# tu-darmstadt-ros-pkg/hector_slam

Measured on AMD Instinct MI355X. Metric: scan-match GN iterations/sec (1081-beam, 2048^2 map), higher is better.
Workload: dtype f32; 1 GPU; configs[2]: batch=4096/GPU concurrent 1081-beam scans (distinct pose+scan pairs), 2048^2 map, 1-level matchData = 6 GN it/scan, starts +-0.15 m / +-0.05 rad (SURVEY 8(d)); batch_per_gpu=4096, global_batch=4096, beams=1081, map=2048, levels=1, parallelism=dp1, parity_mode=library default (HSM_PARITY_AUTO) -> exact summation for this launch, parity_effective=exact

## Files before the change

hector_slam_amd/csrc/gn_match_exact.h:

```cpp
#pragma once
#include "gn_match.h"

namespace hsm {

constexpr int kXRow = 64 + kExactPad;

#ifndef HSM_XBPC
#define HSM_XBPC 15
#endif
#ifndef HSM_XBPC_MAIN
#define HSM_XBPC_MAIN 13
#endif
#ifndef HSM_XBPC_CW
#define HSM_XBPC_CW 6
#endif
constexpr int kXRows = 9;
#ifndef HSM_XOWNER_PRIO_P
#define HSM_XOWNER_PRIO_P 1
#endif
#ifndef HSM_XOWNER_SHIFT
#define HSM_XOWNER_SHIFT 8
#endif
#ifndef HSM_XEP_AHEAD
#define HSM_XEP_AHEAD 2
#endif
#ifndef HSM_XJOB_PRIO
#define HSM_XJOB_PRIO 3
#endif

#ifdef HSM_XTIMELINE
#define HSM_XT(row, slot)                                                                                            \
  do {                                                                                                               \
    if (P.clock_probe != nullptr && blockIdx.x == 0 && lane == 0)                                                    \
      P.clock_probe[((size_t)wave * BPL + (size_t)(row)) * 4 + (slot)] = (unsigned long long)__builtin_readcyclecounter(); \
  } while (0)
#else
#define HSM_XT(row, slot) \
  do {                    \
  } while (0)
#endif

__device__ __forceinline__ void set_prio_uniform(int p) {
  if (p <= 0) __builtin_amdgcn_s_setprio(0);
  else if (p == 1) __builtin_amdgcn_s_setprio(1);
  else if (p == 2) __builtin_amdgcn_s_setprio(2);
  else __builtin_amdgcn_s_setprio(3);
}

template <int NS, int BPL, int BPC = BPL, bool CW = false, bool PROBE = false>
__global__ void __launch_bounds__(64 * (NS + (CW ? 1 : 0)), CW && 5 * BPC + 50 <= 96 ? 5 : 4) gn_match_exact_cached_kernel(const MatchParams P) {
  static_assert(BPC >= 1 && BPC <= BPL, "cached rows are a prefix of the rows");
  constexpr int NC = 9 * NS;
  static_assert(!CW || NC <= 64, "the chain wavefront runs one job per round: lane = chain");
  constexpr int NCP = NC >= 64 ? NC : 64;
  constexpr int NB = NCP % 64 == 0 ? 2 : 3;
  constexpr int kLdsShare = 160 * 1024 / (16 / NS);
  constexpr int kRowsFit = (kLdsShare - NB * NS * kXRows * kXRow * 4 - NC * 4 - 64) / (NS * 512);
  constexpr int RV = BPL <= kRowsFit ? 0 : BPL - kRowsFit;
  static_assert(RV < BPL && RV <= 8, "endpoint rows kept in VGPRs");
  static_assert(64 * (NS + (CW ? 1 : 0)) <= 1024, "one workgroup");
  struct alignas(16) Smem {
    float stage[NB][NS][kXRows][kXRow];
    float runs[NC];
    int nmax;
    f2 pts[NS][BPL - RV][64];
  };
  static_assert(sizeof(Smem) <= kLdsShare, "16 wavefronts per CU");
  __shared__ Smem sm;
  auto& stage = sm.stage;
  auto& runs = sm.runs;
  int& nmax_s = sm.nmax;
  auto& lds_pts = sm.pts;
  static_assert(sizeof(sm.stage) < 65536, "stage rows are addressed through M0[15:0]");
  const int match_blocks = (!CW && P.xp.world > 0) ? P.xp.match_blocks : (int)gridDim.x;
  if (!CW && (int)blockIdx.x >= match_blocks) {
    exchange_wait_unpack(P.xp, (int)blockIdx.x - match_blocks);
    return;
  }
  const int lane = threadIdx.x & 63;
  const int wave = __builtin_amdgcn_readfirstlane((int)(threadIdx.x >> 6));
  const int slot = __builtin_amdgcn_readfirstlane(xcd_block((int)blockIdx.x, match_blocks, P.xcd_chunk) * NS + wave);
  const int scan = (P.perm != nullptr && slot < P.batch) ? __builtin_amdgcn_readfirstlane(P.perm[slot]) : slot;
  const bool chain_wave = CW && wave == NS;
  const bool active = slot < P.batch && !chain_wave;
  int beg = 0, n = 0;
  float pw0 = 0.0f, pw1 = 0.0f, pw2 = 0.0f;
  if (active) {
    n = P.shared_n;
    if (P.offsets) {
      beg = P.offsets[scan];
      n = P.offsets[scan + 1] - beg;
    }
    pw0 = P.begin_world[3 * scan + 0];
    pw1 = P.begin_world[3 * scan + 1];
    pw2 = P.begin_world[3 * scan + 2];
  }
  pw0 = uniform_f32(pw0), pw1 = uniform_f32(pw1), pw2 = uniform_f32(pw2);
  const float b0 = pw0, b1 = pw1, b2 = pw2;
  if (threadIdx.x == 0) nmax_s = 0;
  __syncthreads();
  if (lane == 0 && n > 0) atomicMax(&nmax_s, n);
  __syncthreads();
  const int nmax = nmax_s;
  if (nmax == 0) {
    if (!CW && active && P.xp.world > 0) exchange_post_pose(P.xp, scan, b0, b1, b2);
    if (active && lane == 0) {
      P.out_pose[3 * scan + 0] = b0;
      P.out_pose[3 * scan + 1] = b1;
      P.out_pose[3 * scan + 2] = b2;
    }
    return;
  }
  const int rounds = BPL + (nmax > 64 * BPL ? (nmax - 64 * BPL + 63) >> 6 : 0);
  const int units = rounds * NCP;
  if (CW && chain_wave) {
    __builtin_amdgcn_s_setprio(HSM_XJOB_PRIO);
    const int c = lane < NC ? lane : 0;
    for (int l = P.first_level; l >= P.last_level; --l) {
      const int gn_steps = __builtin_amdgcn_readfirstlane(P.lv[l].gn_steps);
      for (int it = 0; it < gn_steps; ++it) {
        float run = 0.0f;
        for (int k = 0; k < rounds; ++k) {
          asm volatile("s_waitcnt lgkmcnt(0)\n\ts_barrier" ::: "memory");
          const f4v* pa = reinterpret_cast<const f4v*>(&stage[0][0][0][0] + ((k % NB) * NC + c) * kXRow);
          f4v a[4];
#pragma unroll
          for (int q = 0; q < 4; ++q) a[q] = pa[q];
#pragma unroll
          for (int h = 0; h < 8; ++h) {
            const f4v p0 = a[2 * (h & 1)], p1 = a[2 * (h & 1) + 1];
            run += p0.x;
            run += p0.y;
            run += p0.z;
            run += p0.w;
            run += p1.x;
            run += p1.y;
            run += p1.z;
            run += p1.w;
            asm volatile("" : "+v"(run) : : "memory");
            if (h + 2 < 8) a[2 * (h & 1)] = pa[2 * h + 4], a[2 * (h & 1) + 1] = pa[2 * h + 5];
            asm volatile("" ::: "memory");
          }
        }
        if (lane < NC) runs[lane] = run;
        asm volatile("s_waitcnt lgkmcnt(0)\n\ts_barrier" ::: "memory");
      }
    }
    return;
  }
  const unsigned long long probe_t0 = PROBE ? (unsigned long long)__builtin_readcyclecounter() : 0ull;
  const unsigned long long probe_w0 = PROBE ? wall_clock64() : 0ull;
#ifdef HSM_XTIMELINE_WG
  if (P.clock_probe != nullptr && wave == 0 && lane == 0) {
    P.clock_probe[1024 + 4 * (size_t)blockIdx.x + 0] = wall_clock64();
    unsigned xcc;
    asm volatile("s_getreg_b32 %0, hwreg(HW_REG_XCC_ID)" : "=s"(xcc));
    unsigned hwid;
    asm volatile("s_getreg_b32 %0, hwreg(HW_REG_HW_ID)" : "=s"(hwid));
    P.clock_probe[1024 + 4 * (size_t)blockIdx.x + 2] = ((unsigned long long)xcc << 32) | hwid;
  }
#endif
  const float2* __restrict__ pts = P.pts + (n > 0 ? beg : 0);
  f2(*mine)[64] = lds_pts[wave];
  f2 pv[RV > 0 ? RV : 1];
  constexpr int kEpAhead = HSM_XEP_AHEAD < BPL ? HSM_XEP_AHEAD : BPL - 1;
  static_assert(BPL <= 31, "PeelSchedule holds 32 positions per load kind");
  constexpr PeelSchedule kSched = peel_schedule(BPL, kEpAhead);
  const bool peel = P.lv[P.first_level].gn_steps > 0;
  if (!peel) {
#pragma unroll
    for (int k = 0; k < BPL; ++k) {
      const int i = lane + 64 * k;
      const float2 q = i < n ? pts[i] : make_float2(1.0e30f, 1.0e30f);
      if (k < RV)
        pv[k] = f2{q.x, q.y};
      else
        mine[k - RV][lane] = f2{q.x, q.y};
    }
  }
  f4v tq[BPC];
  unsigned toff[BPC];
  Acc9 acc;
  acc.zero();
  float reg_scale = 1.0f;
  int step_no = 0;
  const int owner_phase = (int)((blockIdx.x >> HSM_XOWNER_SHIFT) & 3u);
  const unsigned st_wave = __builtin_amdgcn_readfirstlane((unsigned)(size_t)&stage[0][wave][0][0]);
  for (int l = P.first_level; l >= P.last_level; --l) {
    const LevelView& L = P.lv[l];
    float ex, ey, eth;
    affine_apply(L.mapTworld, pw0, pw1, ex, ey);
    ex = uniform_f32(ex), ey = uniform_f32(ey);
    eth = pw2;
    const float ps = L.pt_scale;
    const int gn_steps = L.gn_steps;
    const LevelRegs R = level_regs<kLayoutQuad>(L);
    const float ratio = ps / reg_scale;
    reg_scale = ps;
    const bool peel_here = peel && l == P.first_level;
#pragma unroll
    for (int k = 0; k < BPL; ++k) {
      if (!peel_here && ratio != 1.0f) {
        if (k < RV)
          pv[k] *= f2{ratio, ratio};
        else
          mine[k - RV][lane] *= f2{ratio, ratio};
      }
      if (k < BPC) toff[k] = 0xffffffffu;
    }
    unsigned zero_off = (unsigned)R.zero_index << 4;
    asm volatile("" : "+v"(zero_off));
    auto gn_step = [&](auto FIRST) {
      constexpr bool kFirst = decltype(FIRST)::value;
#ifdef HSM_XTIMELINE_STEPS
      if (P.clock_probe != nullptr && blockIdx.x == 0 && wave == 0 && lane == 0 && step_no < 32)
        P.clock_probe[(size_t)4 * 31 * 4 + step_no] = (unsigned long long)__builtin_readcyclecounter();
#endif
      f2 pq[kFirst ? BPL : 1];
      auto endpoint_issue = [&](int k) {
        int i = max(min((int)lane_id_now() + 64 * k, n - 1), 0);
        asm volatile("" : "+v"(i));
        const unsigned byte_off = (unsigned)i << 3;
        asm volatile("global_load_dwordx2 %0, %1, %2" : "=v"(pq[kFirst ? k : 0]) : "v"(byte_off), "s"(pts) : "memory");
      };
      if (kFirst) {
#pragma unroll
        for (int k = 0; k <= kEpAhead; ++k) endpoint_issue(k);
      }
      float sinRot, cosRot;
      sincos_f32<true>(eth, sinRot, cosRot);
      const f2 o2 = step_origin(ex, ey);
      const f2 e2 = f2{uniform_f32(o2.x), uniform_f32(o2.y)};
      const f2 cs = f2{uniform_f32(cosRot), uniform_f32(sinRot)}, sc = f2{cs.y, cs.x};
      auto endpoint = [&](int k) -> f2 {
        if (kFirst) {
          wait_vmcnt(kSched.posG[k] - kSched.posE[k] - 1, pq[kFirst ? k : 0]);
          const bool pad = (int)lane_id_now() + 64 * k >= n;
          const f2 q = pq[kFirst ? k : 0];
          const f2 p = f2{(pad ? 1.0e30f : q.x) * ps, (pad ? 1.0e30f : q.y) * ps};
          if (k < RV)
            pv[k < RV ? k : 0] = p;
          else
            mine[k < RV ? 0 : k - RV][lane] = p;
          return p;
        }
        return k < RV ? pv[k < RV ? k : 0] : mine[k < RV ? 0 : k - RV][lane];
      };
      f4v tu[2];
      auto locate = [&](int k, f2 p, BeamRot& r, float& fx, float& fy) {
        r.r.x = cs.x * p.x - sc.x * p.y;
        r.r.y = cs.y * p.x + sc.y * p.y;
        const CellCoord q = cell_coord(R, f2{e2.x + r.r.x, e2.y + r.r.y});
        fx = q.fx;
        fy = q.fy;
        unsigned idx = quad_index(q.ix, q.iy, R.tiles_x, R.sx);
        asm volatile("" : "+v"(idx));
        const unsigned off = q.oob ? zero_off : idx << 4;
        if (k >= BPC) {
          asm volatile("global_load_dwordx4 %[t], %[o], %[b]" : [t] "=v"(tu[k & 1]) : [o] "v"(off), [b] "s"(R.quad) : "memory");
          return;
        }
        const int kc = k < BPC ? k : 0;
        if (kFirst) {
          asm volatile("global_load_dwordx4 %[t], %[o], %[b]" : [t] "=v"(tq[kc]) : [o] "v"(off), [b] "s"(R.quad) : "memory");
          toff[kc] = off;
          return;
        }
        unsigned long long saved;
        asm volatile(
            "v_cmp_ne_u32 vcc, %[o], %[to]\n\t"
            "s_or_b32 vcc_lo, vcc_lo, 1\n\t"
            "s_and_saveexec_b64 %[sv], vcc\n\t"
            "global_load_dwordx4 %[t], %[o], %[b]\n\t"
            "v_mov_b32 %[to], %[o]\n\t"
            "s_mov_b64 exec, %[sv]"
            : [t] "+v"(tq[kc]), [to] "+v"(toff[kc]), [sv] "=&s"(saved)
            : [o] "v"(off), [b] "s"(R.quad)
            : "vcc", "scc", "memory");
      };
      auto texel_ready = [&](int k, bool has_next) {
        f4v& tx = k < BPC ? tq[k < BPC ? k : 0] : tu[k & 1];
        if (kFirst) {
          wait_vmcnt((has_next ? kSched.posG[k + 1] + 1 : kSched.total) - kSched.posG[k] - 1, tx);
        } else if (has_next) {
          asm volatile("s_waitcnt vmcnt(1)" : "+v"(tx) : : "memory");
        } else {
          asm volatile("s_waitcnt vmcnt(0)" : "+v"(tx) : : "memory");
        }
      };
      auto beam_terms4 = [&](float i0, float i1, float i2, float i3, const BeamRot& r, float fx, float fy, float (&tm)[4]) {
        const float xFacInv = 1.0f - fx, yFacInv = 1.0f - fy;
        const float M = ((i0 * xFacInv + i1 * fx) * (yFacInv)) + ((i2 * xFacInv + i3 * fx) * (fy));
        tm[0] = ((i1 - i0) * xFacInv) + ((i3 - i2) * fx);
        tm[1] = ((i2 - i0) * yFacInv) + ((i3 - i1) * fy);
        tm[2] = 1.0f - M;
        tm[3] = r.r.x * tm[1] - r.r.y * tm[0];
      };
      auto products_of = [&](const float (&tm)[4], float (&pp)[9]) {
        const float gx = tm[0], gy = tm[1], funVal = tm[2], rotDeriv = tm[3];
        pp[0] = gx * funVal, pp[1] = gy * funVal, pp[2] = rotDeriv * funVal;
        pp[3] = gx * gx, pp[4] = gy * gy, pp[5] = rotDeriv * rotDeriv;
        pp[6] = gx * gy, pp[7] = gx * rotDeriv, pp[8] = gy * rotDeriv;
      };
      auto products = [&](float i0, float i1, float i2, float i3, const BeamRot& r, float fx, float fy, float (&pp)[9]) {
        float tm[4];
        beam_terms4(i0, i1, i2, i3, r, fx, fy, tm);
        products_of(tm, pp);
      };
      auto stage_write = [&](int k, const float (&pp)[9]) {
        const int buf = k % NB;
        const unsigned m0v = st_wave + (unsigned)buf * (NS * kXRows * kXRow * 4);
        asm volatile(
            "s_mov_b32 m0, %[m]\n\t"
            "s_nop 0\n\t"
            "ds_write_addtid_b32 %[p0] offset:%[o0]\n\t"
            "ds_write_addtid_b32 %[p1] offset:%[o1]\n\t"
            "ds_write_addtid_b32 %[p2] offset:%[o2]\n\t"
            "ds_write_addtid_b32 %[p3] offset:%[o3]\n\t"
            "ds_write_addtid_b32 %[p4] offset:%[o4]\n\t"
            "ds_write_addtid_b32 %[p5] offset:%[o5]\n\t"
            "ds_write_addtid_b32 %[p6] offset:%[o6]\n\t"
            "ds_write_addtid_b32 %[p7] offset:%[o7]\n\t"
            "ds_write_addtid_b32 %[p8] offset:%[o8]"
            :
            : [m] "s"(m0v), [p0] "v"(pp[0]), [p1] "v"(pp[1]), [p2] "v"(pp[2]), [p3] "v"(pp[3]), [p4] "v"(pp[4]), [p5] "v"(pp[5]), [p6] "v"(pp[6]),
              [p7] "v"(pp[7]), [p8] "v"(pp[8]), [o0] "n"(0 * kXRow * 4), [o1] "n"(1 * kXRow * 4), [o2] "n"(2 * kXRow * 4),
              [o3] "n"(3 * kXRow * 4), [o4] "n"(4 * kXRow * 4), [o5] "n"(5 * kXRow * 4), [o6] "n"(6 * kXRow * 4),
              [o7] "n"(7 * kXRow * 4), [o8] "n"(8 * kXRow * 4)
            : "memory");
      };
      auto produce = [&](int k, float i0, float i1, float i2, float i3, const BeamRot& r, float fx, float fy) {
        float pp[9];
        products(i0, i1, i2, i3, r, fx, fy, pp);
        stage_write(k, pp);
      };
      auto chain_job = [&](int j, int k) {
        constexpr bool kOneJob = NCP == 64;
        const int u = kOneJob ? 64 * k + lane : 64 * j + lane_id_now();
        const bool prev = kOneJob ? false : u < k * NCP;
        const int ku = prev ? k - 1 : k, c = kOneJob ? lane : u - ku * NCP;
        if ((kOneJob || u < units) && c < NC) {
          const int buf = prev ? (k + NB - 1) % NB : k % NB;
          float run = ku == 0 ? 0.0f : runs[c];
          const f4v* pa = reinterpret_cast<const f4v*>(&stage[0][0][0][0] + (buf * NC + c) * kXRow);
          f4v a[4];
#pragma unroll
          for (int q = 0; q < 4; ++q) a[q] = pa[q];
#pragma unroll
          for (int h = 0; h < 8; ++h) {
            const f4v p0 = a[2 * (h & 1)], p1 = a[2 * (h & 1) + 1];
            run += p0.x;
            run += p0.y;
            run += p0.z;
            run += p0.w;
            run += p1.x;
            run += p1.y;
            run += p1.z;
            run += p1.w;
            asm volatile("" : "+v"(run) : : "memory");
            if (h + 2 < 8) a[2 * (h & 1)] = pa[2 * h + 4], a[2 * (h & 1) + 1] = pa[2 * h + 5];
            asm volatile("" ::: "memory");
          }
          runs[c] = run;
        }
      };
      const int wg_order = (int)((blockIdx.x >> 8) & 3u);
      const int wg_prio = min(wg_order, 2);
      if (!CW) set_prio_uniform(wg_prio);
      const int my_rounds =
          __builtin_amdgcn_readfirstlane((int)((unsigned)(wave + 64 * NS - (step_no + owner_phase) % NS) % (unsigned)NS));
      auto round_done = [&](int k, bool last_round) {
        if (HSM_XOWNER_PRIO_P != 0) __builtin_amdgcn_s_setprio(0);
        if (k < BPL) HSM_XT(k, 0);
        asm volatile("s_waitcnt lgkmcnt(0)\n\ts_barrier" ::: "memory");
        if (k < BPL) HSM_XT(k, 1);
        if (CW) return;
        const int j_lo = (k * NCP) >> 6;
        const int j_hi = last_round ? (units + 63) >> 6 : ((k + 1) * NCP) >> 6;
        if (j_lo >= j_hi) return;
        int mine_now = my_rounds;
        asm volatile("" : "+s"(mine_now));
        if ((int)((unsigned)k % (unsigned)NS) != mine_now) return;
        __builtin_amdgcn_s_setprio(HSM_XJOB_PRIO);
        for (int j = j_lo; j < j_hi; ++j) chain_job(j, k);
        __builtin_amdgcn_s_setprio(HSM_XOWNER_PRIO_P);
        if (k < BPL) HSM_XT(k, 2);
      };
      {
        BeamRot rc, rn;
        float fxc, fyc, fxn = 0.0f, fyn = 0.0f;
        constexpr bool kAhead = !kFirst;
        constexpr bool kBalanced = !CW && NCP == 64 && !kFirst && (BPL < 17 || BPC <= HSM_XBPC_MAIN);
        f2 p_next = f2{0.0f, 0.0f};
        if (kAhead) p_next = endpoint(BPL > 1 ? 1 : 0);
        locate(0, endpoint(0), rc, fxc, fyc);
#pragma unroll
        for (int k = 0; k < BPL; ++k) {
          if (kFirst && k + 1 + kEpAhead < BPL) endpoint_issue(k + 1 + kEpAhead);
          if (kAhead) {
            const f2 p_cur = p_next;
            if (k + 2 < BPL) p_next = endpoint(k + 2);
            if (k + 1 < BPL) locate(k + 1, p_cur, rn, fxn, fyn);
          } else {
            if (k + 1 < BPL) locate(k + 1, endpoint(k + 1), rn, fxn, fyn);
          }
          if (kBalanced) {
            int mine_now = my_rounds;
            asm volatile("" : "+s"(mine_now));
            const int o = (int)((unsigned)(k + NS - mine_now) % (unsigned)NS);
            if (o == 3 && k >= 1) {
              asm volatile("s_waitcnt lgkmcnt(0)\n\ts_barrier" ::: "memory");
            }
            texel_ready(k, k + 1 < BPL);
            const f4v& tx = k < BPC ? tq[k < BPC ? k : 0] : tu[k & 1];
            float pp[9];
            products(tx.x, tx.y, tx.z, tx.w, rc, fxc, fyc, pp);
            if (o >= 2 || k == 0) {
              stage_write(k, pp);
              if (k == 0 && o == 1) asm volatile("s_waitcnt lgkmcnt(0)\n\ts_barrier" ::: "memory");
            } else {
              asm volatile("s_waitcnt lgkmcnt(0)\n\ts_barrier" ::: "memory");
              stage_write(k, pp);
              if (o == 1) {
                __builtin_amdgcn_s_setprio(HSM_XJOB_PRIO);
                chain_job(k - 1, k - 1);
                set_prio_uniform(wg_prio);
                asm volatile("s_waitcnt lgkmcnt(0)\n\ts_barrier" ::: "memory");
              }
            }
            if (k == BPL - 1 && o != 1) {
              asm volatile("s_waitcnt lgkmcnt(0)\n\ts_barrier" ::: "memory");
              if (o == 0) {
                __builtin_amdgcn_s_setprio(HSM_XJOB_PRIO);
                chain_job(k, k);
                set_prio_uniform(wg_prio);
              }
            }
          } else {
            texel_ready(k, k + 1 < BPL);
            {
              const f4v& tx = k < BPC ? tq[k < BPC ? k : 0] : tu[k & 1];
              produce(k, tx.x, tx.y, tx.z, tx.w, rc, fxc, fyc);
            }
            round_done(k, k == BPL - 1 && rounds == BPL);
          }
          rc = rn;
          fxc = fxn;
          fyc = fyn;
        }
      }
      for (int k = BPL; k < rounds; ++k) {
        const int i = 64 * k + lane;
        const float2 p = i < n ? pts[i] : make_float2(1.0e30f, 1.0e30f);
        BeamRot r;
        const BeamSample b = beam_fetch<kLayoutQuad>(R, e2, cs, sc, f2{p.x * ps, p.y * ps}, r);
        produce(k, b.lo.x, b.lo.y, b.hi.x, b.hi.y, r, b.X.y, b.Y.y);
        round_done(k, k == rounds - 1);
      }
      asm volatile("s_waitcnt lgkmcnt(0)\n\ts_barrier" ::: "memory");
      {
        const float* tt = &runs[9 * wave];
        acc.d01 = f2{uniform_f32(tt[0]), uniform_f32(tt[1])};
        acc.d2 = uniform_f32(tt[2]);
        acc.hd = f2{uniform_f32(tt[3]), uniform_f32(tt[4])};
        acc.h22 = uniform_f32(tt[5]);
        acc.h01 = uniform_f32(tt[6]);
        acc.hr = f2{uniform_f32(tt[7]), uniform_f32(tt[8])};
      }
      gn_solve_and_step(acc, ex, ey, eth);
      ex = uniform_f32(ex), ey = uniform_f32(ey), eth = uniform_f32(eth);
    };
    int it = 0;
    if (peel_here) {
      gn_step(std::true_type{});
      ++step_no;
      it = 1;
    }
    for (; it < gn_steps; ++it, ++step_no) gn_step(std::false_type{});
    eth = normalize_angle<true>(eth);
    affine_apply(L.worldTmap, ex, ey, pw0, pw1);
    pw0 = uniform_f32(pw0), pw1 = uniform_f32(pw1), pw2 = uniform_f32(eth);
  }
#if !defined(HSM_XTIMELINE) && !defined(HSM_XTIMELINE_STEPS) && !defined(HSM_XTIMELINE_WG)
  if (PROBE && P.clock_probe != nullptr && blockIdx.x == 0 && wave == 0 && lane == 0) {
    P.clock_probe[0] = probe_t0, P.clock_probe[1] = probe_w0;
    P.clock_probe[2] = (unsigned long long)__builtin_readcyclecounter();
    P.clock_probe[3] = wall_clock64();
  }
#endif
#ifdef HSM_XTIMELINE_STEPS
  if (P.clock_probe != nullptr && blockIdx.x == 0 && wave == 0 && lane == 0 && step_no < 32)
    P.clock_probe[(size_t)4 * 31 * 4 + step_no] = (unsigned long long)__builtin_readcyclecounter();
#endif
#ifdef HSM_XTIMELINE_WG
  if (P.clock_probe != nullptr && wave == 0 && lane == 0) P.clock_probe[1024 + 4 * (size_t)blockIdx.x + 1] = wall_clock64();
#endif
  if (!CW && active && P.xp.world > 0) exchange_post_pose(P.xp, scan, n == 0 ? b0 : pw0, n == 0 ? b1 : pw1, n == 0 ? b2 : pw2);
  if (active && lane == 0) {
    const bool empty = n == 0;
    P.out_pose[3 * scan + 0] = empty ? b0 : pw0;
    P.out_pose[3 * scan + 1] = empty ? b1 : pw1;
    P.out_pose[3 * scan + 2] = empty ? b2 : pw2;
    if (P.out_cov && !empty) {
      float* c = P.out_cov + 9 * scan;
      c[0] = acc.hd.x; c[1] = acc.h01; c[2] = acc.hr.x;
      c[3] = acc.h01; c[4] = acc.hd.y; c[5] = acc.hr.y;
      c[6] = acc.hr.x; c[7] = acc.hr.y; c[8] = acc.h22;
    }
  }
}

}
```

Baseline: 425.2 million GN it/s.

## Triple-buffer stage rows in balanced path and write products before barrier

In the balanced exact-summation path the stage buffer goes from double to triple buffering, and the GEMM-like products are now always written to LDS before the barrier instead of after it for some wavefront offsets. The extra buffer lets a wavefront write row k without first waiting on the barrier that frees row k-2, removing a sync stall on the critical path. In exchange it uses more LDS, so fewer endpoint rows fit in shared memory and more are spilled to VGPRs (the VGPR limit is raised to 12), which raises register pressure. Trace hooks are also added around the barriers and jobs.

```diff
diff --git a/hector_slam_amd/csrc/gn_match_exact.h b/hector_slam_amd/csrc/gn_match_exact.h
--- a/hector_slam_amd/csrc/gn_match_exact.h
+++ b/hector_slam_amd/csrc/gn_match_exact.h
@@ -53,11 +53,12 @@
   constexpr int NC = 9 * NS;
   static_assert(!CW || NC <= 64, "the chain wavefront runs one job per round: lane = chain");
   constexpr int NCP = NC >= 64 ? NC : 64;
-  constexpr int NB = NCP % 64 == 0 ? 2 : 3;
+  constexpr bool kBalancedForm = !CW && NCP == 64 && (BPL < 17 || BPC <= HSM_XBPC_MAIN);
+  constexpr int NB = NCP % 64 == 0 ? (kBalancedForm ? 3 : 2) : 3;
   constexpr int kLdsShare = 160 * 1024 / (16 / NS);
   constexpr int kRowsFit = (kLdsShare - NB * NS * kXRows * kXRow * 4 - NC * 4 - 64) / (NS * 512);
   constexpr int RV = BPL <= kRowsFit ? 0 : BPL - kRowsFit;
-  static_assert(RV < BPL && RV <= 8, "endpoint rows kept in VGPRs");
+  static_assert(RV < BPL && RV <= (kBalancedForm ? 12 : 8), "endpoint rows kept in VGPRs");
   static_assert(64 * (NS + (CW ? 1 : 0)) <= 1024, "one workgroup");
   struct alignas(16) Smem {
     float stage[NB][NS][kXRows][kXRow];
@@ -390,7 +391,7 @@
         BeamRot rc, rn;
         float fxc, fyc, fxn = 0.0f, fyn = 0.0f;
         constexpr bool kAhead = !kFirst;
-        constexpr bool kBalanced = !CW && NCP == 64 && !kFirst && (BPL < 17 || BPC <= HSM_XBPC_MAIN);
+        constexpr bool kBalanced = kBalancedForm && !kFirst;
         f2 p_next = f2{0.0f, 0.0f};
         if (kAhead) p_next = endpoint(BPL > 1 ? 1 : 0);
         locate(0, endpoint(0), rc, fxc, fyc);
@@ -408,33 +409,37 @@
             int mine_now = my_rounds;
             asm volatile("" : "+s"(mine_now));
             const int o = (int)((unsigned)(k + NS - mine_now) % (unsigned)NS);
-            if (o == 3 && k >= 1) {
+            auto meet = [&](int row) {
+              HSM_XT(row, 0);
               asm volatile("s_waitcnt lgkmcnt(0)\n\ts_barrier" ::: "memory");
-            }
+              HSM_XT(row, 1);
+            };
+            auto job = [&](int row) {
+              __builtin_amdgcn_s_setprio(HSM_XJOB_PRIO);
+              chain_job(row, row);
+              set_prio_uniform(wg_prio);
+              HSM_XT(row, 2);
+            };
+            if (o == 3 && k >= 1) meet(k - 1);
             texel_ready(k, k + 1 < BPL);
             const f4v& tx = k < BPC ? tq[k < BPC ? k : 0] : tu[k & 1];
-            float pp[9];
-            products(tx.x, tx.y, tx.z, tx.w, rc, fxc, fyc, pp);
-            if (o >= 2 || k == 0) {
+            {
+              float pp[9];
+              products(tx.x, tx.y, tx.z, tx.w, rc, fxc, fyc, pp);
               stage_write(k, pp);
-              if (k == 0 && o == 1) asm volatile("s_waitcnt lgkmcnt(0)\n\ts_barrier" ::: "memory");
-            } else {
-              asm volatile("s_waitcnt lgkmcnt(0)\n\ts_barrier" ::: "memory");
-              stage_write(k, pp);
-              if (o == 1) {
-                __builtin_amdgcn_s_setprio(HSM_XJOB_PRIO);
-                chain_job(k - 1, k - 1);
-                set_prio_uniform(wg_prio);
-                asm volatile("s_waitcnt lgkmcnt(0)\n\ts_barrier" ::: "memory");
-              }
+            }
+            if (k == 0) {
+              if (o == 1) meet(0);
+            } else if (o == 0) {
+              meet(k - 1);
+            } else if (o == 1) {
+              meet(k - 1);
+              job(k - 1);
+              meet(k);
             }
             if (k == BPL - 1 && o != 1) {
-              asm volatile("s_waitcnt lgkmcnt(0)\n\ts_barrier" ::: "memory");
-              if (o == 0) {
-                __builtin_amdgcn_s_setprio(HSM_XJOB_PRIO);
-                chain_job(k, k);
-                set_prio_uniform(wg_prio);
-              }
+              meet(k);
+              if (o == 0) job(k);
             }
           } else {
             texel_ready(k, k + 1 < BPL);
```

After: 417.7 million GN it/s. 0.982x the previous value.
